# Justin-Huber/SfM-project

Measured on AMD Instinct MI355X. Metric: verified matches/sec (match+RANSAC), higher is better.
Workload: dtype int8 MFMA -> exact int32 (K1), f32 (K2); 1 GPU; cfg4: all 124750 unordered pairs of 500 synthetic images x 4096 128-D u8 SIFT-like descriptors; L2 match (mutual cross check + ratio 4/5) + 8-point RANSAC 4096 hyp/pair (seed 42, Sampson 1 px^2, min 15 inliers); launches of <= 131072 pairs; n_img=500, k=4096, n_hyp=4096, pairs_total=124750, pairs_rank0=124750, launches_rank0=1, parallelism=pair-sharded dp1

## Files before the change

### include/sfmcore.h

```cpp
#ifndef SFMCORE_H
#define SFMCORE_H

#include <stdint.h>

#ifdef __cplusplus
extern "C" {
#endif

#define SFM_OK 0
#define SFM_ERR_INVALID (-1)
#define SFM_ERR_HIP (-2)
#define SFM_ERR_NOMEM (-3)

#define SFM_METRIC_L2 0
#define SFM_METRIC_HAMMING 1

#define SFM_XC_NONE 0
#define SFM_XC_MUTUAL 1
#define SFM_XC_OPENCV 2

typedef struct sfm_ctx sfm_ctx;

typedef struct sfm_match_params {
    int32_t metric;
// ... 167 lines not shown
    double thr;
    uint64_t seed;
} sfm_register_params;

int sfm_register_batch(sfm_ctx* ctx, int32_t n_img, const int32_t* corr_ptr, const double* xy,
                       const double* X, const double* intr, const int32_t* img_id,
                       const sfm_register_params* prm, double* out_cams, int32_t* out_count,
                       int32_t* out_key, uint8_t* out_mask);

typedef struct sfm_orb_params {
    int32_t n_features;
    int32_t n_levels;
    double scale_factor;
    int32_t fast_threshold;
    int32_t _pad;
} sfm_orb_params;

int sfm_orb_batch(sfm_ctx* ctx, const uint8_t* images, int32_t n_img, int32_t H, int32_t W,
                  const sfm_orb_params* prm, float* out_kp, uint8_t* out_desc,
                  int32_t* out_count);

int sfm_vocab_assign(sfm_ctx* ctx, const uint8_t* desc, const int32_t* n_kp, int32_t n_img,
                     int32_t k_max, const uint8_t* vocab, int32_t n_words, int32_t* out_word,
                     int32_t* out_dist);
int sfm_bow_hist(sfm_ctx* ctx, const int32_t* word, const int32_t* n_kp, int32_t n_img,
                 int32_t k_max, int32_t n_words, uint16_t* out_hist);
int sfm_bow_neighbours(sfm_ctx* ctx, const uint16_t* hist, int32_t n_img, int32_t n_words,
                       const int32_t* weight, int32_t k, int32_t* out_nbr, int64_t* out_score);

int sfm_calib_mfma_i8(sfm_ctx* ctx, float target_ms, double* out);

int sfm_match_cert_stats(sfm_ctx* ctx, int32_t enable, uint64_t* out);

int32_t sfm_l2fr_rev_grid(void);

#ifdef __cplusplus
}
#endif
#endif
```

### sfm-project_amd/csrc/capi.hip

```cpp
#include "sfm_internal.h"

static thread_local std::string g_err;

namespace sfm {
void set_error(const std::string& msg) { g_err = msg; }

void* workspace(sfm_ctx* ctx, size_t bytes) {
    ctx->rs_last_w = nullptr;
    ctx->rs_last_pairs = ctx->rs_last_hyp = 0;
    if (bytes <= ctx->ws_bytes) return ctx->ws;
    hipStreamCaptureStatus cap = hipStreamCaptureStatusNone;
    if (hipStreamIsCapturing(ctx->stream, &cap) == hipSuccess && cap != hipStreamCaptureStatusNone) {
        set_error("workspace growth to " + std::to_string(bytes) +
                  " bytes while the context's stream is being captured: run the call once "
                  "uncaptured first so the workspace is sized");
        return nullptr;
    }
    if (ctx->ws) {
        (void)hipStreamSynchronize(ctx->stream);
        (void)hipFree(ctx->ws);
        ctx->ws = nullptr;
        ctx->ws_bytes = 0;
    }
    size_t want = align_up(bytes + bytes / 4, 1 << 20);
    if (hipMalloc(&ctx->ws, want) != hipSuccess) {
        set_error("workspace allocation of " + std::to_string(want) + " bytes failed");
        return nullptr;
    }
    ctx->ws_bytes = want;
    return ctx->ws;
}
}

extern "C" {

const char* sfm_last_error(void) { return g_err.c_str(); }

int32_t sfm_version(void) { return 5; }

int sfm_ctx_create(int32_t device, sfm_ctx** out) {
    SFM_REQUIRE(out != nullptr, "sfm_ctx_create: out is NULL");
    *out = nullptr;
// ... 127 lines not shown
```

### sfm-project_amd/csrc/match_l2fr.hip

```cpp
#include <algorithm>
#include <climits>
#include <cstdlib>

#include "l2fr_records.h"
#include "match_common.h"

namespace {

typedef int v4i __attribute__((ext_vector_type(4)));
typedef int v16i __attribute__((ext_vector_type(16)));
typedef __attribute__((address_space(3))) void lds_void;
typedef const __attribute__((address_space(1))) void gbl_void;

constexpr int D = 128;
#ifndef L2FR_WAVES
#define L2FR_WAVES 8
#endif
constexpr int WAVES = L2FR_WAVES;
constexpr int SCAN_THREADS = 64 * WAVES;
#ifndef L2FR_QT
#define L2FR_QT 4
#endif
constexpr int QT = L2FR_QT;
constexpr int QB = WAVES * QT * 32;
constexpr int SCAN_MIN_WAVES = 8 / QT;
#ifndef L2FR_CHUNK
#define L2FR_CHUNK 256
#endif
constexpr int CHUNK = L2FR_CHUNK;
constexpr int GROUP = 256;
constexpr int NT = CHUNK / 32;
constexpr int NK = D / 32;
constexpr int SLOTS = D / 16;
constexpr int PIECES = CHUNK * D / 1024 / WAVES;
constexpr int RPP = 1024 / D;
constexpr int KALIGN = CHUNK > GROUP ? CHUNK : GROUP;
// ... 36 lines not shown
                                         const int32_t* __restrict__ n_kp, int k_max, int k_pad,
                                         int32_t* __restrict__ norm, int32_t* __restrict__ cinit,
                                         uint8_t* __restrict__ zero_row,
                                         uint4* __restrict__ desc_i8) {
    if (img == 0 && j < D) zero_row[j] = 0;
    if (j >= k_pad) return;
    int nv = 0;
    if (j < k_max) {
        const uint4* p = (const uint4*)(desc + ((size_t)img * k_max + j) * D);
        uint4* o8 = desc_i8 + ((size_t)img * k_max + j) * SLOTS;
#pragma unroll
        for (int q = 0; q < SLOTS; ++q) {
            const uint4 v = p[q];
            const uint4 x = make_uint4(v.x ^ 0x80808080u, v.y ^ 0x80808080u, v.z ^ 0x80808080u,
                                       v.w ^ 0x80808080u);
            o8[q] = x;
            nv = __builtin_amdgcn_sdot4((int)x.x, (int)x.x, nv, false);
            nv = __builtin_amdgcn_sdot4((int)x.y, (int)x.y, nv, false);
            nv = __builtin_amdgcn_sdot4((int)x.z, (int)x.z, nv, false);
            nv = __builtin_amdgcn_sdot4((int)x.w, (int)x.w, nv, false);
        }
    }
    const size_t o = (size_t)img * k_pad + j;
    norm[o] = nv;
    cinit[o] = (j < n_kp[img]) ? -((nv + 1) >> 1) : PAD_INIT;
}

constexpr int REC_R = 4;

#ifndef L2FR_UNIT
#define L2FR_UNIT 2
#endif
constexpr int UNIT = L2FR_UNIT;
__device__ void build_units(const int32_t* __restrict__ pairs, int n_pairs, int n_img,
                            const int32_t* __restrict__ n_kp, int4* __restrict__ uinfo,
                            int32_t* __restrict__ n_units, int* lds) {
    int* cur = lds;
    int* fu = lds + n_img;
    int* ru = lds + 2 * n_img + 1;
    __shared__ int ftot;
    const int tid = threadIdx.x;
    for (int i = tid; i < n_img; i += 1024) cur[i] = 0;
    __syncthreads();
    auto live = [&](int a, int b) { return n_kp[a] > 0 && n_kp[b] > 0; };
    for (int p = tid; p < n_pairs; p += 1024)
        if (live(pairs[2 * p], pairs[2 * p + 1])) atomicAdd(&cur[pairs[2 * p]], 1);
    __syncthreads();
    if (tid == 0) {
        int f = 0, r = 0;
        for (int i = 0; i < n_img; ++i) {
            const int c = cur[i];
            fu[i] = f;
            ru[i] = r;
            f += c / UNIT;
            r += (c % UNIT) != 0;
            cur[i] = 0;
        }
        fu[n_img] = f;
        ru[n_img] = r;
        ftot = f;
        *n_units = f + r;
    }
    __syncthreads();
    for (int t = tid; t < ru[n_img] * UNIT; t += 1024) uinfo[(size_t)ftot * UNIT + t] = make_int4(-1, 0, 0, 0);
    __syncthreads();
    for (int p = tid; p < n_pairs; p += 1024) {
        const int a = pairs[2 * p], b = pairs[2 * p + 1];
        if (!live(a, b)) continue;
        const int k = atomicAdd(&cur[a], 1);
        const int nf = UNIT * (fu[a + 1] - fu[a]);
        const int u = k < nf ? fu[a] + k / UNIT : ftot + ru[a];
        const int jj = k < nf ? k % UNIT : k - nf;
        uinfo[(size_t)u * UNIT + jj] = jj ? make_int4(p, b, n_kp[b], 0)
                                          : make_int4(p, a, b, n_kp[a] | (n_kp[b] << 16));
    }
}

__device__ void order_block(int ob, const int32_t* __restrict__ pairs, int n_pairs, int n_img,
                            int32_t* __restrict__ order,
                            int2* __restrict__ rng, int32_t* __restrict__ n_rng,
                            const int32_t* __restrict__ n_kp, int4* __restrict__ rinfo,
                            int4* __restrict__ sinfo_f, int unit_blk, int4* __restrict__ uinfo,
                            int32_t* __restrict__ n_units, int* hist) {
    if (ob == unit_blk) {
        build_units(pairs, n_pairs, n_img, n_kp, uinfo, n_units, hist);
        return;
    }
    const int tid = threadIdx.x;
    for (int i = tid; i < n_img; i += 1024) hist[i] = 0;
    __syncthreads();
    for (int p = tid; p < n_pairs; p += 1024) atomicAdd(&hist[pairs[2 * p + 1]], 1);
    __syncthreads();
    int* roff = hist + n_img;
    if (tid == 0) {
        int off = 0, nr = 0;
        for (int i = 0; i < n_img; ++i) {
            const int c = hist[i];
            roff[i] = nr;
            nr += (c + REC_R - 1) / REC_R;
            hist[i] = off;
            off += c;
        }
        n_rng[0] = nr;
        n_rng[1] = 0;
    }
    __syncthreads();
    for (int i = tid; i < n_img; i += 1024) {
        const int c = (i + 1 < n_img ? hist[i + 1] : n_pairs) - hist[i];
        for (int k = 0; k < c; k += REC_R)
            rng[roff[i] + k / REC_R] = make_int2(hist[i] + k, min(REC_R, c - k));
    }
    __syncthreads();
    for (int p = tid; p < n_pairs; p += 1024) {
        const int a = pairs[2 * p], b = pairs[2 * p + 1];
        const int slot = atomicAdd(&hist[b], 1);
        order[slot] = p;
        sinfo_f[slot] = make_int4(p, a, b, n_kp[a] | (n_kp[b] << 16));
    }
    __threadfence_block();
    __syncthreads();
    const int nr = *n_rng;
    for (int r = tid; r < nr; r += 1024) {
        const int2 g = rng[r];
#pragma unroll
        for (int e = 0; e < REC_R; ++e) {
            int4 v = make_int4(-1, 0, 0, 0);
            if (e < g.y) {
                const int p = order[g.x + e], a = pairs[2 * p], b = pairs[2 * p + 1];
                v = make_int4(p, a, b, n_kp[a] | (n_kp[b] << 16));
            }
            rinfo[(size_t)r * REC_R + e] = v;
        }
    }
}

__global__ __launch_bounds__(1024) void l2fr_setup_kernel(
    int n_prep, int bpi, const uint8_t* __restrict__ desc, const int32_t* __restrict__ n_kp,
    int k_max, int k_pad, int32_t* __restrict__ norm, int32_t* __restrict__ cinit,
    uint8_t* __restrict__ zero_row, uint4* __restrict__ desc_i8, const int32_t* __restrict__ pairs,
    int n_pairs, int n_img, int32_t* __restrict__ order_f,
    int2* __restrict__ rng, int32_t* __restrict__ n_rng, int4* __restrict__ rinfo,
    int4* __restrict__ sinfo_f, int unit_blk, int4* __restrict__ uinfo,
    int32_t* __restrict__ n_units) {
    extern __shared__ int hist[];
    const int b = (int)blockIdx.x;
    if (b < n_prep) {
        const int img = b / bpi;
        prep_one(img, (b - img * bpi) * 1024 + (int)threadIdx.x, desc, n_kp, k_max, k_pad, norm,
                 cinit, zero_row, desc_i8);
        return;
    }
    order_block(b - n_prep, pairs, n_pairs, n_img, order_f, rng, n_rng, n_kp, rinfo,
                sinfo_f, unit_blk, uinfo, n_units, hist);
}

__device__ __forceinline__ unsigned char classify(int e1, int e2, long long A, int rnum, int rden,
                                                  long long max_dist) {
    const long long d1lo = max(A - 2LL * e1 - 1, 0LL);
    const long long d2hi = e2 > E_VALID ? A - 2LL * e2 : sfm::DIST_INF;
    if (!sfm::ratio_ok(d1lo, d2hi, rnum, rden, true) || (max_dist >= 0 && !(d1lo < max_dist)))
        return ST_DROP;
    return (e2 == e1) ? ST_SLOW : ST_CAND;
}

struct FwdCls {
    const int32_t* norm;
    int rnum, rden;
    long long max_dist;
    rec8* fwd;
    uint8_t* cls;
};

#ifdef L2FR_CLOCK
constexpr int L2FR_CLOCK_SLOTS = 1 << 16;
constexpr int L2FR_CLOCK_W = 24;
__device__ unsigned long long g_l2fr_clock[L2FR_CLOCK_W * L2FR_CLOCK_SLOTS];
#define L2FR_STAMP(i, v) \
    if (!REV && tid == 0 && bid < L2FR_CLOCK_SLOTS) g_l2fr_clock[L2FR_CLOCK_W * (size_t)bid + (i)] = (v)
#else
#define L2FR_STAMP(i, v)
#endif

template <bool REV>
__device__ __forceinline__ void scan_body(
    const unsigned bid, const unsigned n_bid, const int n_list,
    const uint8_t* __restrict__ desc, const int32_t* __restrict__ n_kp, int k_max, int k_pad,
    const int32_t* __restrict__ cinit, const uint8_t* __restrict__ zero_row,
    const int32_t* __restrict__ pairs, int n_qblk, const int32_t* __restrict__ pair_order,
    const int4* __restrict__ sinfo, int n_blk, const int4* __restrict__ qlist,
    const int32_t* __restrict__ qcount, int4* __restrict__ out, FwdCls fc,
    const int32_t* __restrict__ n_units) {
    __shared__ __attribute__((aligned(16))) unsigned char lds0[CHUNK * D + CHUNK * 4];
    __shared__ __attribute__((aligned(16))) unsigned char lds1[CHUNK * D + CHUNK * 4];

    int p, qi, ti, nq, nb, qb;
    int p2 = -1, ti2 = 0, nb2 = 0;
    int pos = 0, kk = 0;
    if (!REV && n_units) {
        const int nu = *n_units;
        const int u8 = (nu + 7) >> 3;
        const int l = (int)(bid >> 3);
        qb = u8 > 0 ? l / u8 : n_qblk;
        pos = (l - qb * u8) * 8 + (int)(bid & 7);
        if (qb >= n_qblk || pos >= nu) return;
        const int4 u = sinfo[(size_t)UNIT * pos];
        asm volatile("" : : "s"(u.x), "s"(u.y), "s"(u.z), "s"(u.w));
        p = u.x;
        qi = u.y;
        ti = u.z;
        nq = u.w & 0xFFFF;
        nb = u.w >> 16;
    } else if (REV) {
        qb = (int)bid / n_list;
        p = pair_order[(int)bid - qb * n_list];
        qi = pairs[2 * p + 1];
        ti = pairs[2 * p];
        nq = qcount[p];
        nb = n_kp[ti];
    } else {
        const int ppx = (int)(n_bid >> 3) / n_qblk;
        const int l = (int)(bid >> 3);
        const int pos = (int)(bid & 7) * ppx + l % ppx;
        qb = l / ppx;
        if (pos >= n_blk) return;
        const int4 u = sinfo[pos];
        asm volatile("" : : "s"(u.x), "s"(u.y), "s"(u.z), "s"(u.w));
        p = u.x;
        qi = u.y;
        ti = u.z;
        nq = u.w & 0xFFFF;
        nb = u.w >> 16;
    }
    if (qb * QB >= nq || nb <= 0) return;
    const int tid = threadIdx.x, wave = tid >> 6, lane = tid & 63, h = lane >> 5, r32 = lane & 31;
    L2FR_STAMP(0, __builtin_amdgcn_s_memrealtime());

    const uint8_t* db = desc + (size_t)ti * k_max * D;
// ... 251 lines not shown
            if (ch + 1 < 16) L2FR_STAMP(4 + ch, __builtin_amdgcn_s_memrealtime());
        }
    };
    int g = 0;
    for (;;) {
        if (g & 1)
            run_pair(lds1, lds0);
        else
            run_pair(lds0, lds1);
        g += n_chunk;
        L2FR_STAMP(19, __builtin_amdgcn_s_memtime());
        L2FR_STAMP(20, __builtin_amdgcn_s_memrealtime());
        if (active) epilogue();
        if (p2 < 0) break;
        p = p2;
        ti = ti2;
        nb = nb2;
        db = db2;
        cib = cib2;
        n_chunk = (nb + CHUNK - 1) / CHUNK;
        find_next();
    }
#ifdef L2FR_CLOCK
    L2FR_STAMP(21, __builtin_amdgcn_s_memrealtime());
    L2FR_STAMP(22, (unsigned)__builtin_amdgcn_s_getreg((31 << 11) | 4));
    L2FR_STAMP(23, (unsigned)__builtin_amdgcn_s_getreg((15 << 11) | 20));
#endif
}

__global__ __launch_bounds__(SCAN_THREADS, SCAN_MIN_WAVES) void l2fr_scan_fwd_kernel(
    const uint8_t* __restrict__ desc, const int32_t* __restrict__ n_kp, int k_max, int k_pad,
    const int32_t* __restrict__ cinit, const uint8_t* __restrict__ zero_row,
    const int32_t* __restrict__ pairs, int n_qblk, const int4* __restrict__ sinfo, int n_blk,
    FwdCls fc, const int32_t* __restrict__ n_units) {
    scan_body<false>(blockIdx.x, gridDim.x, 0, desc, n_kp, k_max, k_pad, cinit, zero_row, pairs, n_qblk,
                     nullptr, sinfo, n_blk, nullptr, nullptr, nullptr, fc, n_units);
}

constexpr int REV_GRID = 1024;
__global__ __launch_bounds__(SCAN_THREADS, SCAN_MIN_WAVES) void l2fr_scan_rev_kernel(
    const uint8_t* __restrict__ desc, const int32_t* __restrict__ n_kp, int k_max, int k_pad,
    const int32_t* __restrict__ cinit, const uint8_t* __restrict__ zero_row,
    const int32_t* __restrict__ pairs, int n_qblk, const int32_t* __restrict__ flist,
    const int32_t* __restrict__ n_flag, const int4* __restrict__ qlist,
    const int32_t* __restrict__ qcount, int4* __restrict__ out) {
    const int nl = *n_flag;
    for (unsigned u = blockIdx.x; u < (unsigned)(nl * n_qblk); u += gridDim.x) {
        scan_body<true>(u, 0, nl, desc, n_kp, k_max, k_pad, cinit, zero_row, pairs, n_qblk, flist,
                        nullptr, 0, qlist, qcount, out, FwdCls{}, nullptr);
        __syncthreads();
    }
}

struct Top2 { long long b1; int j1; long long b2; };

__device__ __forceinline__ Top2 top2_merge(Top2 x, Top2 y) {
    const bool xf = (x.b1 < y.b1) || (x.b1 == y.b1 && x.j1 < y.j1);
    Top2 r;
    r.b1 = xf ? x.b1 : y.b1;
    r.j1 = xf ? x.j1 : y.j1;
    r.b2 = min(min(x.b2, y.b2), xf ? y.b1 : x.b1);
    return r;
}

__device__ Top2 exact_row_scan(const uint4* qrow, const uint8_t* db, const int32_t* normb, int nb,
                               int qnorm, Top2* red) {
    const int tid = threadIdx.x;
    uint4 x[SLOTS];
#pragma unroll
    for (int s = 0; s < SLOTS; ++s) x[s] = qrow[s];
    Top2 m{sfm::DIST_INF, INT_MAX, sfm::DIST_INF};
    for (int j = tid; j < nb; j += 256) {
        const int dot = dot128(x, (const uint4*)(db + (size_t)j * D));
        const long long d = (long long)qnorm + normb[j] - 2LL * dot;
        m = top2_merge(m, Top2{d, j, sfm::DIST_INF});
    }
    red[tid] = m;
    __syncthreads();
    for (int s = 128; s > 0; s >>= 1) {
        if (tid < s) red[tid] = top2_merge(red[tid], red[tid + s]);
        __syncthreads();
    }
// ... 588 lines not shown
        }
        out_match[((size_t)p * k_max + i) * 2] = r.x;
        out_match[((size_t)p * k_max + i) * 2 + 1] = r.y;
        out_dist[(size_t)p * k_max + i] = r.z;
    }
    if (threadIdx.x == 0) out_count[p] = n;
}

}

int sfm_match_l2fr_launch(sfm_ctx* ctx, const uint8_t* desc, const int32_t* n_kp, int32_t n_img,
                          int32_t k_max, const int32_t* pairs, int32_t n_pairs,
                          const sfm_match_params* prm, int32_t* out_count, int32_t* out_match,
                          int32_t* out_dist) {
    hipStream_t st = ctx->stream;
    if (k_max == 0) {
        SFM_HIP_CHECK(hipMemsetAsync(out_count, 0, sizeof(int32_t) * n_pairs, st));
        return SFM_OK;
    }
    const int k_pad = (int)sfm::align_up((size_t)k_max, KALIGN);
    SFM_REQUIRE(k_pad <= KMAX, "sfm_match_batch: L2 matcher needs k_max <= 4096");
    const int n_qblk = (k_max + QB - 1) / QB;
    const size_t tab = (size_t)n_img * k_pad * sizeof(int32_t);
    const size_t recb = (size_t)n_pairs * k_pad * sizeof(int4);
    const size_t cntb = sfm::align_up(sizeof(int32_t) * (size_t)n_pairs, 256);
    const size_t descb = sfm::align_up((size_t)n_img * k_max * D, 256);
    const size_t ordb = sfm::align_up(sizeof(int32_t) * (size_t)n_pairs, 256);
    const size_t clsb = sfm::align_up((size_t)n_pairs * k_pad, 256);
    const int n_rng_max = n_pairs / REC_R + n_img + 1;
    const size_t rngb = sfm::align_up(sizeof(int2) * (size_t)n_rng_max, 256);
    const size_t rinfob = sizeof(int4) * (size_t)n_rng_max * REC_R;
    const size_t sinfob = sfm::align_up(sizeof(int4) * (size_t)n_pairs, 256);
    const size_t uinfob = sfm::align_up(UNIT * sizeof(int4) * (size_t)n_pairs, 256);
    char* ws = (char*)sfm::workspace(ctx, 256 + 2 * tab + 2 * recb + cntb + descb + ordb + clsb +
                                              256 + rngb + rinfob + 256 + sinfob + uinfob + 256 +
                                              cntb);
    if (!ws) return SFM_ERR_NOMEM;
    char* w = ws;
    uint8_t* zero_row = (uint8_t*)w; w += 256;
    int32_t* norm = (int32_t*)w; w += tab;
    int32_t* cinit = (int32_t*)w; w += tab;
    int4* surv = (int4*)w; w += recb;
    int4* rev = (int4*)w; w += recb;
    rec8* fwd = (rec8*)rev;
    rec8* qst = fwd + (size_t)n_pairs * k_pad;
    int32_t* scount = (int32_t*)w; w += cntb;
    uint8_t* desc_i8 = (uint8_t*)w; w += descb;
    int32_t* ord_f = (int32_t*)w; w += ordb;
    uint8_t* cls = (uint8_t*)w; w += clsb;
    int32_t* n_rng = (int32_t*)w; w += 256;
    int32_t* n_flag = n_rng + 1;
    int2* rng = (int2*)w; w += rngb;
    int4* rinfo = (int4*)w; w += rinfob;
    int4* sinfo_f = (int4*)sfm::align_up((size_t)w, 256);
    int4* uinfo = (int4*)((char*)sinfo_f + sinfob);
    int32_t* n_units = (int32_t*)((char*)uinfo + uinfob);
    int32_t* flist = (int32_t*)((char*)n_units + 256);
    static const bool units_env = [] {
        const char* e = getenv("SFM_L2FR_UNITS");
        return !(e && e[0] == '0');
    }();
    const bool units = units_env && (3 * (size_t)n_img + 2) * sizeof(int) <= 65536;
    const int ppx = (n_pairs + 7) / 8;
    const int n_blk = n_pairs;
    const int grid = 8 * ppx * n_qblk;
    const bool mutual = prm->cross_check == SFM_XC_MUTUAL;

    const int unit_blk = units ? 1 : -1;
    const int bpi = (k_pad + 1023) / 1024, n_prep = bpi * n_img;
    hipLaunchKernelGGL(l2fr_setup_kernel, dim3(n_prep + 1 + (units ? 1 : 0)), dim3(1024),
                       ((units ? 3 : 2) * (size_t)n_img + 2) * sizeof(int), st, n_prep, bpi, desc, n_kp,
                       k_max, k_pad, norm, cinit, zero_row, (uint4*)desc_i8, pairs, n_pairs, n_img,
                       ord_f, rng, n_rng, rinfo, sinfo_f, unit_blk, uinfo, n_units);
    SFM_HIP_CHECK(hipGetLastError());
    const FwdCls fc{norm, prm->ratio_num, prm->ratio_den, (long long)prm->max_dist, fwd, cls};
    hipLaunchKernelGGL(l2fr_scan_fwd_kernel, dim3(grid), dim3(SCAN_THREADS), 0, st, desc_i8, n_kp, k_max,
                       k_pad, cinit, zero_row, pairs, n_qblk, (const int4*)(units ? uinfo : sinfo_f),
                       n_blk, fc, (const int32_t*)(units ? n_units : nullptr));
    SFM_HIP_CHECK(hipGetLastError());
    const char* dbg = getenv("SFM_L2FR_DEBUG");
    int dmode = dbg ? atoi(dbg) : 0;
    if (dmode < 1 || dmode > 3) dmode = 0;
    if (dmode == 1) {
        hipLaunchKernelGGL(l2fr_dump_kernel, dim3(n_pairs), dim3(256), 0, st, n_kp, pairs, k_max,
                           k_pad, (const int4*)nullptr, (const rec8*)fwd, (const int32_t*)nullptr,
                           out_count, out_match, out_dist);
        return SFM_OK;
    }
    hipLaunchKernelGGL(l2fr_recover_mfma_kernel, dim3(n_rng_max * (k_pad / GROUP)), dim3(256), 0, st,
                       desc_i8, k_max, k_pad, norm, cinit, (const int4*)rinfo, (const int32_t*)n_rng,
                       (const rec8*)fwd, (const uint8_t*)cls, prm->ratio_num, prm->ratio_den,
                       (long long)prm->max_dist, qst);
    SFM_HIP_CHECK(hipGetLastError());
    const char* ce = getenv("SFM_L2FR_CERT");
    const bool cert = mutual && dmode == 0 && !(ce && ce[0] == '0');
    const char* cc = getenv("SFM_L2FR_CERT_CAP");
    const long long cap = cc ? atoll(cc) : CERT_CAP_DEFAULT;
    unsigned long long* stats = cert && ctx->cert_stats ? ctx->cert_acc : nullptr;
    if (stats)
        SFM_HIP_CHECK(hipMemsetAsync(stats, 0, 3 * sizeof(unsigned long long), st));
    auto tail = !mutual && dmode == 0 ? l2fr_tail_kernel<TAIL_DIRECT>
                : cert                ? l2fr_tail_kernel<TAIL_CERT>
                                      : l2fr_tail_kernel<TAIL_SPILL>;
    hipLaunchKernelGGL(tail, dim3(n_pairs), dim3(256), 0, st, desc_i8, n_kp, k_max, k_pad, norm, pairs,
                       (const rec8*)fwd, (const uint8_t*)cls, qst, prm->ratio_num, prm->ratio_den,
                       (long long)prm->max_dist, cap, surv, scount, flist, n_flag, stats, out_count,
                       out_match, out_dist);
    SFM_HIP_CHECK(hipGetLastError());
    if (!mutual && dmode == 0) return SFM_OK;
    if (dmode == 2) {
        hipLaunchKernelGGL(l2fr_dump_kernel, dim3(n_pairs), dim3(256), 0, st, n_kp, pairs, k_max,
// ... 9 lines not shown
    }
    if (dmode == 3) {
        hipLaunchKernelGGL(l2fr_dump_kernel, dim3(n_pairs), dim3(256), 0, st, n_kp, pairs, k_max,
                           k_pad, (const int4*)rev, (const rec8*)nullptr, (const int32_t*)scount,
                           out_count, out_match, out_dist);
        return SFM_OK;
    }
    hipLaunchKernelGGL(l2fr_final_kernel, dim3(REV_GRID), dim3(256), 0, st, desc_i8, n_kp, k_max, k_pad,
                       norm, cinit, pairs, surv, scount, rev, (const int32_t*)flist,
                       (const int32_t*)n_flag, out_count, out_match, out_dist);
    SFM_HIP_CHECK(hipGetLastError());
    return SFM_OK;
}

extern "C" int32_t sfm_l2fr_rev_grid(void) { return REV_GRID; }

extern "C" int sfm_match_cert_stats(sfm_ctx* ctx, int32_t enable, uint64_t* out) {
    SFM_REQUIRE(ctx, "sfm_match_cert_stats: ctx is NULL");
    SFM_HIP_CHECK(hipSetDevice(ctx->device));
    if (!ctx->cert_acc) {
        SFM_HIP_CHECK(hipMalloc(&ctx->cert_acc, 3 * sizeof(unsigned long long)));
        SFM_HIP_CHECK(hipMemsetAsync(ctx->cert_acc, 0, 3 * sizeof(unsigned long long), ctx->stream));
    }
    if (out) {
        unsigned long long h[3];
        SFM_HIP_CHECK(hipMemcpyAsync(h, ctx->cert_acc, sizeof(h), hipMemcpyDeviceToHost, ctx->stream));
        SFM_HIP_CHECK(hipStreamSynchronize(ctx->stream));
        out[0] = h[0]; out[1] = h[1]; out[2] = h[2];
    }
    ctx->cert_stats = enable ? 1 : 0;
    return SFM_OK;
}

#ifdef L2FR_CLOCK
extern "C" int sfm_debug_l2fr_stamps(unsigned long long* host, int32_t n_blocks) {
    const size_t n = L2FR_CLOCK_W * (size_t)std::min(n_blocks, L2FR_CLOCK_SLOTS);
    SFM_HIP_CHECK(hipDeviceSynchronize());
    SFM_HIP_CHECK(hipMemcpyFromSymbol(host, HIP_SYMBOL(g_l2fr_clock), n * sizeof(unsigned long long)));
    return SFM_OK;
}
#endif
```

### sfm-project_amd/csrc/sfm_internal.h

```cpp
#pragma once
#include <hip/hip_runtime.h>
#include <stdint.h>
#include <string>

#include "../../include/sfmcore.h"

struct sfm_ctx {
    int device = 0;
    hipStream_t own_stream = nullptr;
    hipStream_t stream = nullptr;
    void* ws = nullptr;
    size_t ws_bytes = 0;
    hipEvent_t handoff = nullptr;
    int32_t* pinned = nullptr;
    hipEvent_t poll_ev = nullptr;
    int n_cu = 256;
    int ransac_stats = 0;
    unsigned long long* rs_acc = nullptr;
    const uint32_t* rs_last_w = nullptr;
    int rs_last_pairs = 0, rs_last_hyp = 0;
    int cert_stats = 0;
    unsigned long long* cert_acc = nullptr;
    int ba_nchunk = 0, ba_ntotal = 0;
    int32_t ba_chunk_pt[17] = {0}, ba_chunk_obs[17] = {0};
    const int32_t* ba_cam_bounds = nullptr;
    int ba_nslot = 0, ba_nseg = 0, ba_ninst = 0, ba_nent = 0, ba_ngroup = 0;
    const int32_t *ba_slot_cam = nullptr, *ba_seg = nullptr, *ba_inst = nullptr,
                  *ba_row_ptr = nullptr, *ba_row_ent = nullptr, *ba_sg_ptr = nullptr,
                  *ba_sg = nullptr, *ba_gk = nullptr;
};

namespace sfm {

struct ChunkOff {
    int32_t v[17];
};
__device__ __forceinline__ int chunk_of(int x, int nck, const ChunkOff& off, const ChunkOff& base,
                                        int& a, int& b) {
    int k = 0;
    a = base.v[0];
    b = base.v[1];
#pragma unroll
    for (int i = 1; i < 16; ++i) {
        if (i < nck && x >= off.v[i]) {
            k = i;
            a = base.v[i];
            b = base.v[i + 1];
        }
    }
    return k;
}
__device__ __forceinline__ double chunk_tree16(double (&a)[16]) {
#pragma unroll
    for (int w = 8; w >= 1; w >>= 1)
#pragma unroll
// ... 85 lines not shown
```

### sfm-project_amd/sfmcore.py

```python
from __future__ import annotations

import ctypes as C
import os
import threading

import numpy as np

_HERE = os.path.dirname(os.path.abspath(__file__))
LIB_PATH = os.environ.get("SFMCORE_LIB") or os.path.join(_HERE, "lib", "libsfmcore.so")

METRIC_L2, METRIC_HAMMING = 0, 1
XC_NONE, XC_MUTUAL, XC_OPENCV = 0, 1, 2

EXPORTED = ["sfm_ctx_create", "sfm_ctx_destroy", "sfm_ctx_set_stream", "sfm_ctx_sync",
            "sfm_last_error", "sfm_version", "sfm_match_batch", "sfm_ransac_f_batch",
            "sfm_ba_jtj", "sfm_graph_offsets", "sfm_graph_rows", "sfm_ba_solve", "sfm_ba_cost",
            "sfm_ba_update", "sfm_tracks", "sfm_triangulate", "sfm_register_batch",
            "sfm_ba_fix_params", "sfm_orb_batch", "sfm_ransac_counts", "sfm_ba_solve_stage",
            "sfm_ransac_stats", "sfm_ransac_f_batch_f64", "sfm_graph_rows_packed",
            "sfm_graph_expand", "sfm_match_batch_both", "sfm_ransac_wave_stops",
            "sfm_ba_set_chunks", "sfm_ba_chunk_tree", "sfm_ba_set_schur", "sfm_calib_mfma_i8",
            "sfm_match_cert_stats", "sfm_ransac_h_batch", "sfm_ransac_h_counts",
            "sfm_two_view_pose_batch", "sfm_l2fr_rev_grid", "sfm_triangulate_robust",
            "sfm_triangulate_cam_table", "sfm_vocab_assign", "sfm_bow_hist",
            "sfm_bow_neighbours"]


class SfmCoreError(RuntimeError):
    pass


class MatchParams(C.Structure):
    _fields_ = [("metric", C.c_int32), ("cross_check", C.c_int32), ("ratio_num", C.c_int32),
                ("ratio_den", C.c_int32), ("max_dist", C.c_int64)]


class BaSolveParams(C.Structure):
    _fields_ = [("lam", C.c_double), ("tol", C.c_double), ("max_iter", C.c_int32),
                ("poll", C.c_int32), ("poll_first", C.c_int32)]


class RegisterParams(C.Structure):
    _fields_ = [("n_hyp", C.c_int32), ("refine", C.c_int32), ("thr", C.c_double),
                ("seed", C.c_uint64)]


class OrbParams(C.Structure):
    _fields_ = [("n_features", C.c_int32), ("n_levels", C.c_int32), ("scale_factor", C.c_double),
                ("fast_threshold", C.c_int32), ("_pad", C.c_int32)]


class RansacParams(C.Structure):
    _fields_ = [("n_hyp", C.c_int32), ("min_inliers", C.c_int32), ("thr", C.c_float),
                ("_pad", C.c_int32), ("seed", C.c_uint64)]


class TwoViewPoseParams(C.Structure):
    _fields_ = [("struct_size", C.c_int32), ("min_inliers", C.c_int32), ("wide_key", C.c_float)]
# ... 18 lines not shown
        if _lib is not None:
            return _lib
        import torch
        if not os.path.exists(path):
            if os.path.exists("/opt/rocm/bin/hipcc"):
                from build_lib import build
                build()
            if not os.path.exists(path):
                raise SfmCoreError(f"libsfmcore.so not found at {path}; run __graft_entry__.build()")
        L = C.CDLL(path)
        vp, i32, i64, f64 = C.c_void_p, C.c_int32, C.c_int64, C.c_double
        L.sfm_ctx_create.argtypes = [i32, C.POINTER(vp)]
        L.sfm_ctx_destroy.argtypes = [vp]
        L.sfm_ctx_set_stream.argtypes = [vp, vp]
        L.sfm_ctx_sync.argtypes = [vp]
        L.sfm_last_error.restype = C.c_char_p
        L.sfm_version.restype = i32
        L.sfm_match_batch.argtypes = [vp, vp, vp, i32, i32, i32, vp, i32, C.POINTER(MatchParams),
                                      vp, vp, vp]
        L.sfm_match_batch_both.argtypes = L.sfm_match_batch.argtypes
        L.sfm_ransac_f_batch.argtypes = [vp, vp, i32, i32, vp, i32, vp, vp,
                                         C.POINTER(RansacParams), vp, vp, vp, vp, vp]
        L.sfm_ransac_f_batch_f64.argtypes = L.sfm_ransac_f_batch.argtypes
        L.sfm_ransac_counts.argtypes = [vp, vp, i32, i32, vp, i32, vp, vp,
                                        C.POINTER(RansacParams), vp, vp, vp, vp]
        L.sfm_ransac_h_batch.argtypes = L.sfm_ransac_f_batch.argtypes
        L.sfm_ransac_h_counts.argtypes = [vp, vp, i32, i32, vp, i32, vp, vp,
                                          C.POINTER(RansacParams), vp, vp, vp]
        L.sfm_two_view_pose_batch.argtypes = [vp, vp, i32, i32, vp, i32, vp, vp, vp, vp, vp,
                                              C.POINTER(TwoViewPoseParams), vp, vp, vp, vp, vp]
        L.sfm_ransac_stats.argtypes = [vp, i32, vp]
        L.sfm_ransac_wave_stops.argtypes = [vp, i32, i32, vp]
        L.sfm_match_cert_stats.argtypes = [vp, i32, vp]
        L.sfm_l2fr_rev_grid.argtypes = []
        L.sfm_l2fr_rev_grid.restype = i32
        L.sfm_calib_mfma_i8.argtypes = [vp, C.c_float, vp]
        L.sfm_ba_jtj.argtypes = [vp, i32, vp, vp, i32, vp, i32, vp, vp, vp, vp, vp, vp, f64, vp,
                                 vp, vp, vp, vp, vp, vp]
        L.sfm_ba_solve.argtypes = [vp, i32, i32, i32, vp, vp, vp, vp, vp, vp, vp, vp, vp, vp,
                                   C.POINTER(BaSolveParams), vp, vp, vp]
        L.sfm_ba_solve_stage.argtypes = [vp, i32, i32, i32, i32, i32, vp, vp, vp, vp, vp, vp, vp,
                                         vp, vp, vp, C.POINTER(BaSolveParams), vp, vp, vp, vp, vp]
        L.sfm_ba_cost.argtypes = [vp, i32, vp, vp, i32, vp, i32, vp, vp, vp, f64, vp]
        L.sfm_ba_update.argtypes = [vp, i32, vp, vp, i32, vp, vp, vp, vp]
        L.sfm_ba_fix_params.argtypes = [vp, i32, i32, vp, vp, vp, vp, vp]
        L.sfm_ba_set_chunks.argtypes = [vp, i32, vp, vp, i32, vp]
        L.sfm_ba_set_schur.argtypes = [vp, i32, vp, i32, vp, i32, vp, vp, i32, vp, i32, vp, vp, vp]
        L.sfm_ba_chunk_tree.argtypes = [vp, i32, i64, vp, vp]
        L.sfm_orb_batch.argtypes = [vp, vp, i32, i32, i32, C.POINTER(OrbParams), vp, vp, vp]
        L.sfm_register_batch.argtypes = [vp, i32, vp, vp, vp, vp, vp, C.POINTER(RegisterParams),
                                         vp, vp, vp, vp]
        L.sfm_triangulate.argtypes = [vp, i32, vp, vp, i32, vp, vp, vp, vp, vp]
        L.sfm_triangulate_robust.argtypes = [vp, i32, vp, vp, i32, vp, vp, vp, vp,
                                             C.POINTER(TriangulateRobustParams), vp, vp, vp, vp]
        L.sfm_triangulate_cam_table.argtypes = [vp, i32, vp, vp, vp]
        L.sfm_tracks.argtypes = [vp, i32, vp, i32, vp, i64, vp, i32, vp, vp, vp, vp]
        L.sfm_graph_offsets.argtypes = [vp, i32, vp, i32, vp]
        L.sfm_graph_rows.argtypes = [vp, i32, i32, i32, vp, vp, vp, vp, i32, vp, vp]
        L.sfm_graph_rows_packed.argtypes = [vp, i32, i32, vp, vp, vp, vp, i32, vp, vp]
        L.sfm_graph_expand.argtypes = [vp, i32, i32, vp, vp, vp, vp, vp]
        L.sfm_vocab_assign.argtypes = [vp, vp, vp, i32, i32, vp, i32, vp, vp]
        L.sfm_bow_hist.argtypes = [vp, vp, vp, i32, i32, i32, vp]
        L.sfm_bow_neighbours.argtypes = [vp, vp, i32, i32, vp, i32, vp, vp]
        for name in EXPORTED:
            getattr(L, name).restype = getattr(L, name).restype or C.c_int
        _lib = L
# ... 284 lines not shown
                                          == inl_count.shape[0] == P):
            raise SfmCoreError("two_view_pose_batch: intr must have one row per image and "
                               "count / match / mask / inl_count one per pair")
        if not 0.0 <= float(min_angle_deg) <= 90.0:
            raise SfmCoreError("two_view_pose_batch: min_angle_deg must lie in [0, 90]")
        dev = kps.device
        if out is None:
            out = dict(E=torch.empty((P, 9), dtype=torch.float64, device=dev),
                       R=torch.empty((P, 9), dtype=torch.float64, device=dev),
                       t=torch.empty((P, 3), dtype=torch.float64, device=dev),
                       stat=torch.empty((P, 8), dtype=torch.int32, device=dev),
                       median_key=torch.empty(P, dtype=torch.float32, device=dev))
        prm = TwoViewPoseParams(C.sizeof(TwoViewPoseParams), int(min_inliers),
                                float(angle_key(min_angle_deg)))
        self._bind_stream()
        _check(self.lib.sfm_two_view_pose_batch(
            self.handle, _ptr(kps), n_img, k_max, _ptr(pairs), P, _ptr(count), _ptr(match),
            _ptr(mask), _ptr(inl_count), _ptr(intr), C.byref(prm), _ptr(out["E"]), _ptr(out["R"]),
            _ptr(out["t"]), _ptr(out["stat"]), _ptr(out["median_key"])))
        return out

    def ransac_stats(self, enable=True, read=False):
        out = (C.c_uint64 * 3)()
        self._bind_stream()
        _check(self.lib.sfm_ransac_stats(self.handle, 1 if enable else 0, out if read else None))
        return (int(out[0]), int(out[1]), int(out[2])) if read else None

    def match_cert_stats(self, enable=True, read=False):
        out = (C.c_uint64 * 3)()
        self._bind_stream()
        _check(self.lib.sfm_match_cert_stats(self.handle, 1 if enable else 0,
                                             out if read else None))
        return (int(out[0]), int(out[1]), int(out[2])) if read else None

    def l2fr_rev_grid(self):
        return int(self.lib.sfm_l2fr_rev_grid())

    def ransac_wave_stops(self, n_pairs, n_hyp):
        out = np.zeros((n_pairs, n_hyp // 64), np.uint32)
        self._bind_stream()
        _check(self.lib.sfm_ransac_wave_stops(self.handle, int(n_pairs), int(n_hyp),
                                              out.ctypes.data_as(C.c_void_p)))
        return out

    def calib_mfma_i8(self, target_ms=200.0):
        out = np.zeros(4, np.float64)
        self._bind_stream()
        _check(self.lib.sfm_calib_mfma_i8(self.handle, float(target_ms),
                                          out.ctypes.data_as(C.c_void_p)))
        return {"ms": float(out[0]), "tops": float(out[1]), "clock_ghz": float(out[2]),
                "frac_nominal": float(out[3])}

    def graph_rows(self, pair_base, count, match, inl_count, mask, min_inliers=15,
                   return_offsets=False, packed=False):
        torch = self.torch
        P, k_max = mask.shape
        dev = mask.device
        offs = torch.empty(P + 1, dtype=torch.int64, device=dev)
        self._bind_stream()
        _check(self.lib.sfm_graph_offsets(self.handle, P, _ptr(inl_count), int(min_inliers),
                                          _ptr(offs)))
        n = int(offs[P].item())
        rows = torch.empty((n,) if packed else (n, 3), dtype=torch.int32, device=dev)
        if n and packed:
            _check(self.lib.sfm_graph_rows_packed(self.handle, P, k_max, _ptr(count),
                                                  _ptr(match), _ptr(mask), _ptr(inl_count),
# ... 350 lines not shown
```

Before: 268.7 million verified matches/s.

## Group L2 match units by partner-image key and window-order blocks across XCDs

Adds a key-sorted unit builder that groups pairs by (b/2, a) so each unit shares descriptor image a and neighbouring b images. It also adds a windowed block-to-item ordering so blocks landing on the same XCD process nearby units and query blocks together. This mode is picked by default when the descriptor footprint exceeds the aggregate L2 size. The aim is better L2 reuse of descriptor tiles in the forward scan, at the cost of a heavier single-block setup pass that does serial scans in LDS. A debug API for dumping the unit mapping is included.

```diff
diff --git a/include/sfmcore.h b/include/sfmcore.h
--- a/include/sfmcore.h
+++ b/include/sfmcore.h
@@ -223,6 +223,9 @@
 
 int sfm_match_cert_stats(sfm_ctx* ctx, int32_t enable, uint64_t* out);
 
+int sfm_match_l2fr_units(sfm_ctx* ctx, int32_t* info, int32_t* out_uinfo, int32_t* out_bid,
+                         int32_t cap_units);
+
 int32_t sfm_l2fr_rev_grid(void);
 
 #ifdef __cplusplus
diff --git a/sfm-project_amd/csrc/capi.hip b/sfm-project_amd/csrc/capi.hip
--- a/sfm-project_amd/csrc/capi.hip
+++ b/sfm-project_amd/csrc/capi.hip
@@ -8,6 +8,7 @@
 void* workspace(sfm_ctx* ctx, size_t bytes) {
     ctx->rs_last_w = nullptr;
     ctx->rs_last_pairs = ctx->rs_last_hyp = 0;
+    ctx->l2fr_ws = nullptr;
     if (bytes <= ctx->ws_bytes) return ctx->ws;
     hipStreamCaptureStatus cap = hipStreamCaptureStatusNone;
     if (hipStreamIsCapturing(ctx->stream, &cap) == hipSuccess && cap != hipStreamCaptureStatusNone) {
diff --git a/sfm-project_amd/csrc/l2fr_order.h b/sfm-project_amd/csrc/l2fr_order.h
--- /dev/null
+++ b/sfm-project_amd/csrc/l2fr_order.h
@@ -0,0 +1,38 @@
+#pragma once
+#include "l2fr_records.h"
+
+namespace l2fr {
+
+constexpr int ORD_XCDS = 8;
+constexpr int ORD_WIN = 32;
+
+struct Item { int unit, qb; };
+
+L2FR_HD int order_item(unsigned bid, int n_items) {
+    const int rows = (n_items + ORD_XCDS - 1) / ORD_XCDS;
+    const int l = (int)(bid / ORD_XCDS), x = (int)(bid % ORD_XCDS);
+    if (l >= rows) return -1;
+    const int w = l / ORD_WIN;
+    const int width = rows - w * ORD_WIN < ORD_WIN ? rows - w * ORD_WIN : ORD_WIN;
+    const int item = w * (ORD_XCDS * ORD_WIN) + x * width + (l - w * ORD_WIN);
+    return item < n_items ? item : -1;
+}
+
+L2FR_HD unsigned order_bid(int item, int n_items) {
+    const int rows = (n_items + ORD_XCDS - 1) / ORD_XCDS;
+    const int w = item / (ORD_XCDS * ORD_WIN);
+    const int width = rows - w * ORD_WIN < ORD_WIN ? rows - w * ORD_WIN : ORD_WIN;
+    const int rem = item - w * (ORD_XCDS * ORD_WIN);
+    const int x = rem / width, l = w * ORD_WIN + rem % width;
+    return (unsigned)l * ORD_XCDS + (unsigned)x;
+}
+
+L2FR_HD Item order_decode(unsigned bid, int n_units, int n_qblk) {
+    const int item = order_item(bid, n_units * n_qblk);
+    Item it;
+    it.unit = item < 0 ? -1 : item / n_qblk;
+    it.qb = item < 0 ? 0 : item % n_qblk;
+    return it;
+}
+
+}
diff --git a/sfm-project_amd/csrc/match_l2fr.hip b/sfm-project_amd/csrc/match_l2fr.hip
--- a/sfm-project_amd/csrc/match_l2fr.hip
+++ b/sfm-project_amd/csrc/match_l2fr.hip
@@ -2,6 +2,7 @@
 #include <climits>
 #include <cstdlib>
 
+#include "l2fr_order.h"
 #include "l2fr_records.h"
 #include "match_common.h"
 
@@ -104,6 +105,8 @@
 #define L2FR_UNIT 2
 #endif
 constexpr int UNIT = L2FR_UNIT;
+enum { L2FR_UNITS_OFF = 0, L2FR_UNITS_A = 1, L2FR_UNITS_KEY_RR = 2, L2FR_UNITS_KEY = 3 };
+constexpr size_t L2FR_L2_BYTES = 8u * (4u << 20);
 __device__ void build_units(const int32_t* __restrict__ pairs, int n_pairs, int n_img,
                             const int32_t* __restrict__ n_kp, int4* __restrict__ uinfo,
                             int32_t* __restrict__ n_units, int* lds) {
@@ -148,14 +151,188 @@
     }
 }
 
+__device__ __forceinline__ void block_scan2(int& f, int& s, int* wsum, int* tot) {
+    const int tid = threadIdx.x, lane = tid & 63, wave = tid >> 6;
+    int fi = f, si = s;
+#pragma unroll
+    for (int d = 1; d < 64; d <<= 1) {
+        const int pf = __shfl_up(fi, d), ps = __shfl_up(si, d);
+        if (lane >= d) { fi += pf; si += ps; }
+    }
+    if (lane == 63) { wsum[wave] = fi; wsum[16 + wave] = si; }
+    __syncthreads();
+    int bf = 0, bs = 0, tf = 0, tsum = 0;
+    for (int w = 0; w < 16; ++w) {
+        const int a = wsum[w], b = wsum[16 + w];
+        bf += w < wave ? a : 0;
+        bs += w < wave ? b : 0;
+        tf += a;
+        tsum += b;
+    }
+    f = bf + fi - f;
+    s = bs + si - s;
+    if (tid == 0) {
+        tot[0] = tf;
+        tot[1] = tsum;
+    }
+    __syncthreads();
+}
+
+__host__ __device__ inline size_t units_key_lds(int n_img) {
+    const size_t n_key = ((size_t)n_img + 1) >> 1;
+    return 2 * (size_t)n_img + 1 + 16 * n_key + n_key + 1;
+}
+__device__ void build_units_key(const int32_t* __restrict__ pairs, int n_pairs, int n_img,
+                                const int32_t* __restrict__ n_kp, int4* __restrict__ uinfo,
+                                int32_t* __restrict__ n_units, int32_t* __restrict__ ws, int* lds) {
+    const int n_key = (n_img + 1) >> 1;
+    int* aoff = lds;
+    int* cur = aoff + n_img + 1;
+    int* wk = cur + n_img;
+    int* kpre = wk + 16 * n_key;
+    int32_t* by_a = ws;
+    int32_t* by_b = ws + n_pairs;
+    int32_t* sp = ws + 2 * (size_t)n_pairs;
+    int32_t* sc = ws + 3 * (size_t)n_pairs;
+    int32_t* lead = by_a;
+    __shared__ int wsum[32], tot[2];
+    const int tid = threadIdx.x, lane = tid & 63, wave = tid >> 6;
+    for (int i = tid; i < n_img; i += 1024) cur[i] = 0;
+    for (int i = tid; i < 16 * n_key; i += 1024) wk[i] = 0;
+    __syncthreads();
+    auto live = [&](int a, int b) { return n_kp[a] > 0 && n_kp[b] > 0; };
+    for (int p = tid; p < n_pairs; p += 1024)
+        if (live(pairs[2 * p], pairs[2 * p + 1])) atomicAdd(&cur[pairs[2 * p]], 1);
+    __syncthreads();
+    if (tid == 0) {
+        int off = 0;
+        for (int i = 0; i < n_img; ++i) {
+            const int c = cur[i];
+            aoff[i] = off;
+            cur[i] = off;
+            off += c;
+        }
+        aoff[n_img] = off;
+    }
+    __syncthreads();
+    const int n_live = aoff[n_img];
+    if (n_live == 0) {
+        if (tid == 0) *n_units = 0;
+        return;
+    }
+    auto wave_of = [&](int a) { return (int)((long long)aoff[a] * 16 / n_live); };
+    for (int p = tid; p < n_pairs; p += 1024) {
+        const int a = pairs[2 * p], b = pairs[2 * p + 1];
+        if (!live(a, b)) continue;
+        const int slot = atomicAdd(&cur[a], 1);
+        by_a[slot] = p;
+        by_b[slot] = b;
+        atomicAdd(&wk[wave_of(a) * n_key + (b >> 1)], 1);
+    }
+    __syncthreads();
+    for (int k = tid; k < n_key; k += 1024) {
+        int t = 0;
+        for (int w = 0; w < 16; ++w) t += wk[w * n_key + k];
+        kpre[k] = t;
+    }
+    __syncthreads();
+    if (tid == 0) {
+        int off = 0;
+        for (int k = 0; k < n_key; ++k) {
+            const int c = kpre[k];
+            kpre[k] = off;
+            off += c;
+        }
+        kpre[n_key] = off;
+    }
+    __syncthreads();
+    for (int k = tid; k < n_key; k += 1024) {
+        int run = kpre[k];
+        for (int w = 0; w < 16; ++w) {
+            const int c = wk[w * n_key + k];
+            wk[w * n_key + k] = run;
+            run += c;
+        }
+    }
+    __threadfence_block();
+    __syncthreads();
+    for (int a = 0; a < n_img; ++a) {
+        const int s = aoff[a], e = aoff[a + 1];
+        if (s == e || wave_of(a) != wave) continue;
+        for (int i0 = s; i0 < e; i0 += 256) {
+            int pp[4], bb[4];
+#pragma unroll
+            for (int j = 0; j < 4; ++j) {
+                const int i = i0 + 64 * j + lane;
+                pp[j] = i < e ? by_a[i] : -1;
+                bb[j] = i < e ? by_b[i] : 0;
+            }
+#pragma unroll
+            for (int j = 0; j < 4; ++j) {
+                if (pp[j] < 0) continue;
+                const int k = bb[j] >> 1;
+                const int slot = atomicAdd(&wk[wave * n_key + k], 1);
+                sp[slot] = pp[j];
+                sc[slot] = (k * n_img + a) * 2 + (bb[j] & 1);
+            }
+        }
+    }
+    __threadfence_block();
+    __syncthreads();
+    const int per = (n_live + 1023) / 1024;
+    const int lo = min(tid * per, n_live), hi = min(lo + per, n_live);
+    int o0 = 0;
+    auto run = [&](int i) { return sc[i] >> 1; };
+    if (lo < hi)
+        for (int j = lo; j > 0 && run(j - 1) == run(lo); --j) ++o0;
+    int nf = 0, ns = 0;
+    {
+        int o = o0;
+        for (int i = lo; i < hi; ++i) {
+            if (i > lo) o = run(i) == run(i - 1) ? o + 1 : 0;
+            if (o & 1) continue;
+            const bool full = i + 1 < n_live && run(i + 1) == run(i);
+            nf += full;
+            ns += !full;
+        }
+    }
+    block_scan2(nf, ns, wsum, tot);
+    const int ftot = tot[0], nu = ftot + tot[1];
+    if (tid == 0) *n_units = nu;
+    int o = o0;
+    for (int i = lo; i < hi; ++i) {
+        if (i > lo) o = run(i) == run(i - 1) ? o + 1 : 0;
+        if (o & 1) continue;
+        const bool full = i + 1 < n_live && run(i + 1) == run(i);
+        lead[full ? nf++ : ftot + ns++] = i;
+    }
+    __threadfence_block();
+    __syncthreads();
+    for (int u = tid; u < nu; u += 1024) {
+        const int i = lead[u];
+        const int c = sc[i], p = sp[i];
+        const int k = (c >> 1) / n_img, a = (c >> 1) - k * n_img, b = 2 * k + (c & 1);
+        uinfo[(size_t)u * UNIT] = make_int4(p, a, b, n_kp[a] | (n_kp[b] << 16));
+        int4 v = make_int4(-1, 0, 0, 0);
+        if (u < ftot) {
+            const int b2 = 2 * k + (sc[i + 1] & 1);
+            v = make_int4(sp[i + 1], b2, n_kp[b2], 0);
+        }
+        uinfo[(size_t)u * UNIT + 1] = v;
+    }
+}
+
 __device__ void order_block(int ob, const int32_t* __restrict__ pairs, int n_pairs, int n_img,
                             int32_t* __restrict__ order,
                             int2* __restrict__ rng, int32_t* __restrict__ n_rng,
                             const int32_t* __restrict__ n_kp, int4* __restrict__ rinfo,
                             int4* __restrict__ sinfo_f, int unit_blk, int4* __restrict__ uinfo,
-                            int32_t* __restrict__ n_units, int* hist) {
+                            int32_t* __restrict__ n_units, int32_t* __restrict__ unit_ws, int* hist) {
     if (ob == unit_blk) {
-        build_units(pairs, n_pairs, n_img, n_kp, uinfo, n_units, hist);
+        if (unit_ws)
+            build_units_key(pairs, n_pairs, n_img, n_kp, uinfo, n_units, unit_ws, hist);
+        else
+            build_units(pairs, n_pairs, n_img, n_kp, uinfo, n_units, hist);
         return;
     }
     const int tid = threadIdx.x;
@@ -213,7 +390,7 @@
     int n_pairs, int n_img, int32_t* __restrict__ order_f,
     int2* __restrict__ rng, int32_t* __restrict__ n_rng, int4* __restrict__ rinfo,
     int4* __restrict__ sinfo_f, int unit_blk, int4* __restrict__ uinfo,
-    int32_t* __restrict__ n_units) {
+    int32_t* __restrict__ n_units, int32_t* __restrict__ unit_ws) {
     extern __shared__ int hist[];
     const int b = (int)blockIdx.x;
     if (b < n_prep) {
@@ -223,7 +400,7 @@
         return;
     }
     order_block(b - n_prep, pairs, n_pairs, n_img, order_f, rng, n_rng, n_kp, rinfo,
-                sinfo_f, unit_blk, uinfo, n_units, hist);
+                sinfo_f, unit_blk, uinfo, n_units, unit_ws, hist);
 }
 
 __device__ __forceinline__ unsigned char classify(int e1, int e2, long long A, int rnum, int rden,
@@ -261,7 +438,7 @@
     const int32_t* __restrict__ pairs, int n_qblk, const int32_t* __restrict__ pair_order,
     const int4* __restrict__ sinfo, int n_blk, const int4* __restrict__ qlist,
     const int32_t* __restrict__ qcount, int4* __restrict__ out, FwdCls fc,
-    const int32_t* __restrict__ n_units) {
+    const int32_t* __restrict__ n_units, const int win_order) {
     __shared__ __attribute__((aligned(16))) unsigned char lds0[CHUNK * D + CHUNK * 4];
     __shared__ __attribute__((aligned(16))) unsigned char lds1[CHUNK * D + CHUNK * 4];
 
@@ -270,11 +447,18 @@
     int pos = 0, kk = 0;
     if (!REV && n_units) {
         const int nu = *n_units;
-        const int u8 = (nu + 7) >> 3;
-        const int l = (int)(bid >> 3);
-        qb = u8 > 0 ? l / u8 : n_qblk;
-        pos = (l - qb * u8) * 8 + (int)(bid & 7);
-        if (qb >= n_qblk || pos >= nu) return;
+        if (win_order) {
+            const l2fr::Item it = l2fr::order_decode(bid, nu, n_qblk);
+            if (it.unit < 0) return;
+            pos = it.unit;
+            qb = it.qb;
+        } else {
+            const int u8 = (nu + 7) >> 3;
+            const int l = (int)(bid >> 3);
+            qb = u8 > 0 ? l / u8 : n_qblk;
+            pos = (l - qb * u8) * 8 + (int)(bid & 7);
+            if (qb >= n_qblk || pos >= nu) return;
+        }
         const int4 u = sinfo[(size_t)UNIT * pos];
         asm volatile("" : : "s"(u.x), "s"(u.y), "s"(u.z), "s"(u.w));
         p = u.x;
@@ -592,9 +776,9 @@
     const uint8_t* __restrict__ desc, const int32_t* __restrict__ n_kp, int k_max, int k_pad,
     const int32_t* __restrict__ cinit, const uint8_t* __restrict__ zero_row,
     const int32_t* __restrict__ pairs, int n_qblk, const int4* __restrict__ sinfo, int n_blk,
-    FwdCls fc, const int32_t* __restrict__ n_units) {
+    FwdCls fc, const int32_t* __restrict__ n_units, int win_order) {
     scan_body<false>(blockIdx.x, gridDim.x, 0, desc, n_kp, k_max, k_pad, cinit, zero_row, pairs, n_qblk,
-                     nullptr, sinfo, n_blk, nullptr, nullptr, nullptr, fc, n_units);
+                     nullptr, sinfo, n_blk, nullptr, nullptr, nullptr, fc, n_units, win_order);
 }
 
 constexpr int REV_GRID = 1024;
@@ -607,7 +791,7 @@
     const int nl = *n_flag;
     for (unsigned u = blockIdx.x; u < (unsigned)(nl * n_qblk); u += gridDim.x) {
         scan_body<true>(u, 0, nl, desc, n_kp, k_max, k_pad, cinit, zero_row, pairs, n_qblk, flist,
-                        nullptr, 0, qlist, qcount, out, FwdCls{}, nullptr);
+                        nullptr, 0, qlist, qcount, out, FwdCls{}, nullptr, 0);
         __syncthreads();
     }
 }
@@ -1262,9 +1446,10 @@
     const size_t rinfob = sizeof(int4) * (size_t)n_rng_max * REC_R;
     const size_t sinfob = sfm::align_up(sizeof(int4) * (size_t)n_pairs, 256);
     const size_t uinfob = sfm::align_up(UNIT * sizeof(int4) * (size_t)n_pairs, 256);
+    const size_t unitb = sfm::align_up(4 * sizeof(int32_t) * (size_t)n_pairs, 256);
     char* ws = (char*)sfm::workspace(ctx, 256 + 2 * tab + 2 * recb + cntb + descb + ordb + clsb +
                                               256 + rngb + rinfob + 256 + sinfob + uinfob + 256 +
-                                              cntb);
+                                              cntb + unitb);
     if (!ws) return SFM_ERR_NOMEM;
     char* w = ws;
     uint8_t* zero_row = (uint8_t*)w; w += 256;
@@ -1286,27 +1471,46 @@
     int4* uinfo = (int4*)((char*)sinfo_f + sinfob);
     int32_t* n_units = (int32_t*)((char*)uinfo + uinfob);
     int32_t* flist = (int32_t*)((char*)n_units + 256);
-    static const bool units_env = [] {
-        const char* e = getenv("SFM_L2FR_UNITS");
-        return !(e && e[0] == '0');
-    }();
-    const bool units = units_env && (3 * (size_t)n_img + 2) * sizeof(int) <= 65536;
+    int32_t* unit_ws = (int32_t*)((char*)flist + cntb);
+    const char* ue = getenv("SFM_L2FR_UNITS");
+    int umode = !ue || !ue[0] ? (descb > L2FR_L2_BYTES ? L2FR_UNITS_KEY : L2FR_UNITS_A)
+                : ue[0] == '0' ? L2FR_UNITS_OFF
+                : ue[0] == 'a' ? L2FR_UNITS_A
+                : ue[0] == 'p' ? L2FR_UNITS_KEY_RR
+                               : L2FR_UNITS_KEY;
+    if ((umode == L2FR_UNITS_KEY || umode == L2FR_UNITS_KEY_RR) &&
+        (UNIT != 2 || units_key_lds(n_img) * sizeof(int) > 65536))
+        umode = L2FR_UNITS_A;
+    if (umode == L2FR_UNITS_A && (3 * (size_t)n_img + 2) * sizeof(int) > 65536) umode = L2FR_UNITS_OFF;
+    const bool units = umode != L2FR_UNITS_OFF;
+    const bool by_key = umode == L2FR_UNITS_KEY || umode == L2FR_UNITS_KEY_RR;
     const int ppx = (n_pairs + 7) / 8;
     const int n_blk = n_pairs;
     const int grid = 8 * ppx * n_qblk;
     const bool mutual = prm->cross_check == SFM_XC_MUTUAL;
+    ctx->l2fr_ws = ws;
+    ctx->l2fr_uinfo = units ? uinfo : nullptr;
+    ctx->l2fr_n_units = n_units;
+    ctx->l2fr_umode = umode;
+    ctx->l2fr_n_qblk = n_qblk;
+    ctx->l2fr_grid = grid;
+    ctx->l2fr_n_pairs = n_pairs;
 
     const int unit_blk = units ? 1 : -1;
     const int bpi = (k_pad + 1023) / 1024, n_prep = bpi * n_img;
+    const size_t setup_lds = std::max(by_key ? units_key_lds(n_img) : 0,
+                                      (umode == L2FR_UNITS_A ? 3 : 2) * (size_t)n_img + 2) * sizeof(int);
     hipLaunchKernelGGL(l2fr_setup_kernel, dim3(n_prep + 1 + (units ? 1 : 0)), dim3(1024),
-                       ((units ? 3 : 2) * (size_t)n_img + 2) * sizeof(int), st, n_prep, bpi, desc, n_kp,
+                       setup_lds, st, n_prep, bpi, desc, n_kp,
                        k_max, k_pad, norm, cinit, zero_row, (uint4*)desc_i8, pairs, n_pairs, n_img,
-                       ord_f, rng, n_rng, rinfo, sinfo_f, unit_blk, uinfo, n_units);
+                       ord_f, rng, n_rng, rinfo, sinfo_f, unit_blk, uinfo, n_units,
+                       by_key ? unit_ws : (int32_t*)nullptr);
     SFM_HIP_CHECK(hipGetLastError());
     const FwdCls fc{norm, prm->ratio_num, prm->ratio_den, (long long)prm->max_dist, fwd, cls};
     hipLaunchKernelGGL(l2fr_scan_fwd_kernel, dim3(grid), dim3(SCAN_THREADS), 0, st, desc_i8, n_kp, k_max,
                        k_pad, cinit, zero_row, pairs, n_qblk, (const int4*)(units ? uinfo : sinfo_f),
-                       n_blk, fc, (const int32_t*)(units ? n_units : nullptr));
+                       n_blk, fc, (const int32_t*)(units ? n_units : nullptr),
+                       umode == L2FR_UNITS_KEY ? 1 : 0);
     SFM_HIP_CHECK(hipGetLastError());
     const char* dbg = getenv("SFM_L2FR_DEBUG");
     int dmode = dbg ? atoi(dbg) : 0;
@@ -1382,6 +1586,44 @@
     return SFM_OK;
 }
 
+extern "C" int sfm_match_l2fr_units(sfm_ctx* ctx, int32_t* info, int32_t* out_uinfo,
+                                    int32_t* out_bid, int32_t cap_units) {
+    SFM_REQUIRE(ctx && info, "sfm_match_l2fr_units: ctx or info is NULL");
+    SFM_REQUIRE(ctx->l2fr_ws && ctx->l2fr_ws == ctx->ws,
+                "sfm_match_l2fr_units: the last call on ctx that used the workspace is no "
+                "ratio-path call");
+    SFM_HIP_CHECK(hipSetDevice(ctx->device));
+    int32_t nu = 0;
+    if (ctx->l2fr_uinfo) {
+        SFM_HIP_CHECK(hipMemcpyAsync(&nu, ctx->l2fr_n_units, sizeof(nu), hipMemcpyDeviceToHost,
+                                     ctx->stream));
+        SFM_HIP_CHECK(hipStreamSynchronize(ctx->stream));
+    }
+    const int n_qblk = ctx->l2fr_n_qblk;
+    info[0] = nu;
+    info[1] = n_qblk;
+    info[2] = ctx->l2fr_grid;
+    info[3] = ctx->l2fr_umode;
+    info[4] = UNIT;
+    info[5] = ctx->l2fr_n_pairs;
+    const int n = std::min(nu, cap_units);
+    if (n > 0 && out_uinfo) {
+        SFM_HIP_CHECK(hipMemcpyAsync(out_uinfo, ctx->l2fr_uinfo, sizeof(int4) * UNIT * (size_t)n,
+                                     hipMemcpyDeviceToHost, ctx->stream));
+        SFM_HIP_CHECK(hipStreamSynchronize(ctx->stream));
+    }
+    if (out_bid) {
+        const int u8 = (nu + 7) >> 3;
+        for (int u = 0; u < n; ++u)
+            for (int qb = 0; qb < n_qblk; ++qb)
+                out_bid[(size_t)u * n_qblk + qb] =
+                    ctx->l2fr_umode == L2FR_UNITS_KEY
+                        ? (int32_t)l2fr::order_bid(u * n_qblk + qb, nu * n_qblk)
+                        : (qb * u8 + u / 8) * 8 + u % 8;
+    }
+    return SFM_OK;
+}
+
 #ifdef L2FR_CLOCK
 extern "C" int sfm_debug_l2fr_stamps(unsigned long long* host, int32_t n_blocks) {
     const size_t n = L2FR_CLOCK_W * (size_t)std::min(n_blocks, L2FR_CLOCK_SLOTS);
diff --git a/sfm-project_amd/csrc/sfm_internal.h b/sfm-project_amd/csrc/sfm_internal.h
--- a/sfm-project_amd/csrc/sfm_internal.h
+++ b/sfm-project_amd/csrc/sfm_internal.h
@@ -21,6 +21,10 @@
     int rs_last_pairs = 0, rs_last_hyp = 0;
     int cert_stats = 0;
     unsigned long long* cert_acc = nullptr;
+    const void* l2fr_ws = nullptr;
+    const void* l2fr_uinfo = nullptr;
+    const int32_t* l2fr_n_units = nullptr;
+    int l2fr_umode = 0, l2fr_n_qblk = 0, l2fr_grid = 0, l2fr_n_pairs = 0;
     int ba_nchunk = 0, ba_ntotal = 0;
     int32_t ba_chunk_pt[17] = {0}, ba_chunk_obs[17] = {0};
     const int32_t* ba_cam_bounds = nullptr;
diff --git a/sfm-project_amd/sfmcore.py b/sfm-project_amd/sfmcore.py
--- a/sfm-project_amd/sfmcore.py
+++ b/sfm-project_amd/sfmcore.py
@@ -23,7 +23,7 @@
             "sfm_match_cert_stats", "sfm_ransac_h_batch", "sfm_ransac_h_counts",
             "sfm_two_view_pose_batch", "sfm_l2fr_rev_grid", "sfm_triangulate_robust",
             "sfm_triangulate_cam_table", "sfm_vocab_assign", "sfm_bow_hist",
-            "sfm_bow_neighbours"]
+            "sfm_bow_neighbours", "sfm_match_l2fr_units"]
 
 
 class SfmCoreError(RuntimeError):
@@ -108,6 +108,7 @@
         L.sfm_ransac_stats.argtypes = [vp, i32, vp]
         L.sfm_ransac_wave_stops.argtypes = [vp, i32, i32, vp]
         L.sfm_match_cert_stats.argtypes = [vp, i32, vp]
+        L.sfm_match_l2fr_units.argtypes = [vp, vp, vp, vp, i32]
         L.sfm_l2fr_rev_grid.argtypes = []
         L.sfm_l2fr_rev_grid.restype = i32
         L.sfm_calib_mfma_i8.argtypes = [vp, C.c_float, vp]
@@ -458,6 +459,21 @@
         _check(self.lib.sfm_match_cert_stats(self.handle, 1 if enable else 0,
                                              out if read else None))
         return (int(out[0]), int(out[1]), int(out[2])) if read else None
+
+    def match_l2fr_units(self):
+        info = np.zeros(6, np.int32)
+        self._bind_stream()
+        vp = C.c_void_p
+        _check(self.lib.sfm_match_l2fr_units(self.handle, info.ctypes.data_as(vp), None, None, 0))
+        nu, nq = int(info[0]), int(info[1])
+        uinfo = np.zeros((nu, int(info[4]), 4), np.int32)
+        bid = np.zeros((nu, nq), np.int32)
+        if nu:
+            _check(self.lib.sfm_match_l2fr_units(self.handle, info.ctypes.data_as(vp),
+                                                 uinfo.ctypes.data_as(vp), bid.ctypes.data_as(vp),
+                                                 nu))
+        return dict(n_units=nu, n_qblk=nq, grid=int(info[2]), mode=int(info[3]),
+                    n_pairs=int(info[5]), uinfo=uinfo, bid=bid)
 
     def l2fr_rev_grid(self):
         return int(self.lib.sfm_l2fr_rev_grid())
```

After: 269.3 million verified matches/s (median of 6 runs). Within noise of the previous version (+0.2%).
